# neeek2303/EMOPortraits

Hardware: AMD Instinct MI355X
Metric: reenactment frames/sec @512x512, 1-src->N-driver (higher is better)
Workload: dtype f32

## Files before the change

emoportraits_amd/csrc/conv_inst_f16x2_up2.hip:

```cpp
#include "conv_dispatch.h"
#include "conv_igemm_bf16x3.h"
#include "conv_split_pair_common.h"

struct ConvCfgUp2 {
  static constexpr int BM = 64, TM = 2, TP = 2, KC = 16, NPL = 2;
  static constexpr int TRL = 2, TWL = 64;
  static constexpr int PR = TRL + 2, NQ = TWL / 4, NQ1 = NQ + 1;
  static constexpr int SUB = ((PR * NQ1 + 4 + 11) / 16) * 16 + 4;
  static constexpr int CHS = 4 * SUB, NG = 2, QPG = 128, NHQ = 2 * PR;
  static constexpr int WPLANE = 2 * BM;
  static constexpr int WTAP = NPL * WPLANE;
  static constexpr int WST = 8 * WTAP;
  static constexpr int WST_BYTES = WST * 16;
  static constexpr int PPL = NG * CHS, PBUF = NPL * PPL;
  static constexpr int OFF_P = 0, OFF_W = 2 * PBUF, OFF_SCT = OFF_W + 2 * WST;
  static constexpr int SCT = 1024;
  static constexpr int OFF_BIAS_F = OFF_SCT * 4 + 2 * SCT;
  static constexpr int EPI_CS = 4 * 132 + 4;
  static constexpr int LDS_BYTES = (OFF_BIAS_F + BM) * 4;
  static_assert(32 * EPI_CS <= OFF_SCT * 4, "the epilogue image lives in the patch and kernel buffers");
  static_assert(WST_BYTES == 32 * 1024, "eight 1 KiB pieces per wave and half-stage");
  static_assert(PR * NQ + NHQ <= QPG, "one interior quad or one halo pixel per thread and stage");
  static_assert(LDS_BYTES <= 160 * 1024, "LDS");
};

__global__ __launch_bounds__(256) __attribute__((amdgpu_waves_per_eu(1, 1)))
void conv_igemm_f16x2_up2_kernel(const ConvArgs a) {
  using Cfg = ConvCfgUp2;
  using opx8 = halfx8;
  constexpr int NPL = 2, NPROD = 3;
  constexpr int BM = Cfg::BM, TM = Cfg::TM, TP = Cfg::TP, KC = Cfg::KC;
  constexpr int PR = Cfg::PR, NQ = Cfg::NQ, NQ1 = Cfg::NQ1, SUB = Cfg::SUB, CHS = Cfg::CHS, QPG = Cfg::QPG;
  constexpr int NHQ = Cfg::NHQ, PPL = Cfg::PPL, PBUF = Cfg::PBUF;
  constexpr bool UPS = false;
  constexpr int TW = Cfg::TWL, TWS = Cfg::TWL;

  extern __shared__ __attribute__((aligned(16))) float smem[];

  const int tid = threadIdx.x;
  const int lane = tid & 63;
  const int wave = __builtin_amdgcn_readfirstlane(tid >> 6);
  const int half = lane >> 5, l32 = lane & 31;
  const int wq = wave & 1;
  const int p0 = (wave >> 1) * TP * 32;
  float sat_m = 0.0f;

  const int HW = a.H * a.W;
  const bool has_affine = a.scale != nullptr;
  const float in_scale = a.in_scale;
  constexpr float CLAMP_HI = 65504.0f;
  const float clamp_lo = a.relu_in ? 0.0f : -CLAMP_HI;
  const int nst = a.n_cchunks;
  const int nptiles = a.tiles_x * a.tiles_y;

  const int q_u = tid % QPG;
  const int q_g = __builtin_amdgcn_readfirstlane(tid / QPG);
  const bool is_quad = q_u < PR * NQ;
  const int hq = q_u - PR * NQ;
  const bool is_halo = !is_quad && hq < NHQ;
  const int h_side = hq & 1;
  const int q_r = is_quad ? q_u / NQ : (is_halo ? hq >> 1 : 0);
  const int q_c = is_quad ? q_u - q_r * NQ : 0;
  int q_slb[4];
#pragma unroll
  for (int i = 0; i < 4; ++i) {
    const int dump = q_g * CHS + i * SUB + PR * NQ1 + (q_u & 3);
    const int own = is_quad ? q_g * CHS + i * SUB + q_r * NQ1 + q_c : q_g * CHS + h_side * SUB + q_r * NQ1 + NQ;
    q_slb[i] = ((is_quad || (is_halo && i == (h_side ? 0 : 3))) ? own : dump) * 16;
  }

  floatx16 acc_lo[2][TM][TP], acc_hi[2][TM][TP];

  const int q8 = a.n_work >> 3, r8 = a.n_work & 7;
  const int xcd = blockIdx.x & 7;
  const int n_mine = q8 + (xcd < r8 ? 1 : 0);
  const int l_base = xcd < r8 ? xcd * (q8 + 1) : r8 * (q8 + 1) + (xcd - r8) * q8;
  const int l_stride = (gridDim.x + 7) >> 3;
#define EMO_U_WPTR(c_, k_, p_) (reinterpret_cast<const char*>(a.wpk) + ((long)((c_) * nst + (k_)) * 2 + (p_)) * Cfg::WST_BYTES)

  const int a_off = (half * BM + l32) * 16;
  EMO_P_DECLARE_B_OFF()

  const char* const lds_c = reinterpret_cast<const char*>(smem);
  char* const lds_w = reinterpret_cast<char*>(smem);
  opx8 fa_[2][NPL][TM], fb_[2][NPL][TP];
#define EMO_U_LOAD_FRAGS_PLANE(set_, pl_, hb_, pbyte_, a_, b_)                                        \
  {                                                                                                   \
    _Pragma("unroll") for (int i = 0; i < TM; ++i)                                                    \
      fa_[set_][pl_][i] = *reinterpret_cast<const opx8*>(lds_c + a_off + (Cfg::OFF_W + (hb_) * Cfg::WST + \
          ((wq * 4 + (a_) * 2 + (b_)) * NPL + (pl_)) * Cfg::WPLANE + i * 32) * 16);                   \
    _Pragma("unroll") for (int j = 0; j < TP; ++j)                                                    \
      fb_[set_][pl_][j] = *reinterpret_cast<const opx8*>(lds_c + (EMO_P_B_OFF(j, (hb_) + (a_), wq + (b_)) + (pbyte_)) + ((pl_) * PPL) * 16); \
  }

  float* const sct = smem + Cfg::OFF_SCT * 4;
  const unsigned smem_lds = (unsigned)(size_t)(__attribute__((address_space(3))) char*)reinterpret_cast<char*>(smem);
  const unsigned lane16 = (unsigned)lane * 16u;

  floatx4 qv[8];
  float q_lo, q_hi;
  int q_tix;
  floatx4 q_sc, q_sh;
  opx8 cv_h, cv_m;
  emo_intx4 xrs = emo_raw_buffer(a.x);
  unsigned usoff[8];
#pragma unroll
  for (int u = 0; u < 8; ++u) usoff[u] = (unsigned)__builtin_amdgcn_readfirstlane((int)((unsigned)u * (unsigned)HW * 4u));
  unsigned lq_off = 0;
  bool lq_ok = false;
  unsigned q_vo;
#define EMO_U_ISSUE_BEGIN(st_)                                                                        \
  {                                                                                                   \
    const int c0_ = (st_) * KC + q_g * 8;                                                             \
    const bool cv_ = c0_ < a.Cin;                                                                     \
    const int cs_ = cv_ ? c0_ : 0;                                                                    \
    const bool keep_ = lq_ok && cv_;                                                                  \
    q_lo = keep_ ? clamp_lo : 0.0f;                                                                   \
    q_hi = keep_ ? CLAMP_HI : 0.0f;                                                                   \
    q_vo = lq_off + (unsigned)cs_ * (unsigned)HW * 4u;                                                \
    q_tix = (has_affine ? cs_ : (cs_ & (Cfg::SCT - 1))) >> 2;                                         \
  }
#define EMO_U_ISSUE_LOADS(u0_, u1_)                                                                   \
  { _Pragma("unroll") for (int u = (u0_); u < (u1_); u += 2) emo_bload4x2_pinned(xrs, q_vo, usoff[u], usoff[u + 1], qv[u], qv[u + 1]); }
#define EMO_U_HALF_TABLE(hf_)                                                                         \
  {                                                                                                   \
    const floatx4* t4_ = reinterpret_cast<const floatx4*>(sct) + q_tix + (hf_);                       \
    q_sc = t4_[0]; q_sh = t4_[Cfg::SCT / 4];                                                          \
  }
#define EMO_U_TOUCH_QUAD() { _Pragma("unroll") for (int u = 0; u < 8; ++u) emo_touch4(qv[u]); }
#define EMO_U_CONV_PIXEL(pbyte_, i_)                                                                  \
  {                                                                                                   \
    _Pragma("unroll") for (int hf_ = 0; hf_ < 2; ++hf_) {                                             \
      EMO_U_HALF_TABLE(hf_)                                                                           \
      float t_[4];                                                                                    \
      _Pragma("unroll") for (int k = 0; k < 4; ++k)                                                   \
        t_[k] = __fmaf_rn(qv[4 * hf_ + k][i_], q_sc[k], q_sh[k]);                                     \
      sat_m = __builtin_fmaxf(__builtin_fmaxf(sat_m, __builtin_fabsf(t_[0])), __builtin_fabsf(t_[1])); \
      sat_m = __builtin_fmaxf(__builtin_fmaxf(sat_m, __builtin_fabsf(t_[2])), __builtin_fabsf(t_[3])); \
      _Pragma("unroll") for (int k = 0; k < 4; k += 2)                                                \
        emo_split_f16x2_pair(__builtin_amdgcn_fmed3f(t_[k], q_lo, q_hi), __builtin_amdgcn_fmed3f(t_[k + 1], q_lo, q_hi), \
                             cv_h, cv_m, 4 * hf_ + k);                                                \
    }                                                                                                 \
    char* d_ = lds_w + (q_slb[i_] + (pbyte_));                                                        \
    *reinterpret_cast<opx8*>(d_) = cv_h;                                                              \
    *reinterpret_cast<opx8*>(d_ + PPL * 16) = cv_m;                                                   \
  }
#define EMO_U_DMA_PIECE(ptr_, wb_, k_)                                                                \
  {                                                                                                   \
    const int j_ = wave + 4 * (k_);                                                                   \
    emo_dma16_pinned_s((ptr_) + j_ * 1024, lane16, smem_lds + (unsigned)((Cfg::OFF_W + (wb_) * Cfg::WST) * 16 + j_ * 1024)); \
  }

  constexpr int PA3[3] = {1, 0, 0}, PB3[3] = {0, 1, 0};
  constexpr int NTE = Cfg::SCT / 256;

  for (int idx8 = blockIdx.x >> 3; idx8 < n_mine; idx8 += l_stride) {
    const int l_ = l_base + idx8;
    const int cotile = __builtin_amdgcn_readfirstlane(l_ % a.n_cotiles);
    const int rest_ = l_ / a.n_cotiles;
    const int it_n = __builtin_amdgcn_readfirstlane(rest_ / nptiles);
    const int lt_ = rest_ - it_n * nptiles;
    const int x0 = __builtin_amdgcn_readfirstlane((lt_ % a.tiles_x) * Cfg::TWL);
    const int y0 = __builtin_amdgcn_readfirstlane((lt_ / a.tiles_x) * Cfg::TRL);
    {
      const int q_y_ = y0 - 1 + q_r;
      const int q_x_ = is_quad ? x0 + 4 * q_c : (h_side ? x0 + TWS : x0 - 4);
      lq_ok = (is_quad || is_halo) && (unsigned)q_y_ < (unsigned)a.H && q_x_ >= 0 && q_x_ < a.W;
      lq_off = lq_ok ? (unsigned)(q_y_ * a.W + q_x_) * 4u : 0u;
    }
    xrs = emo_raw_buffer(a.x + (long)it_n * a.Cin * HW);

#pragma unroll
    for (int u = 0; u < 8; ++u) asm volatile("" : "=v"(qv[u]));
    asm volatile("" : "=v"(cv_h));
    asm volatile("" : "=v"(cv_m));
    {
      const char* const w0_ = EMO_U_WPTR(cotile, 0, 0);
#pragma unroll
      for (int k = 0; k < 8; ++k) EMO_U_DMA_PIECE(w0_, 0, k)
      const char* const w1_ = EMO_U_WPTR(cotile, 0, 1);
      EMO_U_DMA_PIECE(w1_, 1, 0)
      EMO_U_DMA_PIECE(w1_, 1, 1)
    }
    EMO_U_ISSUE_BEGIN(0)
    EMO_U_ISSUE_LOADS(0, 8)
#pragma unroll
    for (int k = 0; k < NTE; ++k) {
      const int c = tid + 256 * k;
      if (c < min(a.Cin, Cfg::SCT)) {
        const bool real = has_affine;
        sct[c] = (real ? a.scale[(long)it_n * a.Cin + c] : 1.0f) * in_scale;
        sct[Cfg::SCT + c] = (real ? a.shift[(long)it_n * a.Cin + c] : 0.0f) * in_scale;
      }
    }
    if (tid < BM) smem[Cfg::OFF_BIAS_F + tid] = a.bias != nullptr ? a.bias[cotile * BM + tid] : 0.0f;
    EMO_P_WAIT(0);
    EMO_U_TOUCH_QUAD()
    __syncthreads();
#pragma unroll
    for (int i = 0; i < 4; ++i) EMO_U_CONV_PIXEL(Cfg::OFF_P * 16, i)
    EMO_U_ISSUE_BEGIN(nst > 1 ? 1 : 0)
    EMO_U_ISSUE_LOADS(0, 8)
    EMO_P_BARRIER(0);
    EMO_U_TOUCH_QUAD()

#pragma unroll
    for (int c = 0; c < 2; ++c)
#pragma unroll
      for (int i = 0; i < TM; ++i)
#pragma unroll
        for (int j = 0; j < TP; ++j)
#pragma unroll
          for (int r = 0; r < 16; ++r) { acc_lo[c][i][j][r] = 0.0f; acc_hi[c][i][j][r] = 0.0f; }
#pragma unroll
    for (int pl = 0; pl < NPL; ++pl) EMO_U_LOAD_FRAGS_PLANE(0, pl, 0, Cfg::OFF_P * 16, 0, 0)
    int pp = 0;
    for (int cg = 0; cg < nst; ++cg) {
      const int pcur_b = (Cfg::OFF_P + pp * PBUF) * 16, pnxt_b = (Cfg::OFF_P + (pp ^ 1) * PBUF) * 16;
      const bool last_ = cg + 1 >= nst;
#pragma unroll
      for (int h = 0; h < 2; ++h) {
        const bool have1_ = h == 0 || !last_, have2_ = !last_;
        const char* const dma1 = EMO_U_WPTR(cotile, h == 0 ? cg : cg + 1, h ^ 1);
        const char* const dma2 = EMO_U_WPTR(cotile, cg + 1, h);
        if (EMO_CONV_SETPRIO) __builtin_amdgcn_s_setprio(1);
#pragma unroll
        for (int gs = 0; gs < 4; ++gs) {
          const int fcur = (h * 4 + gs) & 1, fnxt = fcur ^ 1;
          if (gs == 3) { EMO_P_BARRIER(0); }
          if (gs == 3 && h == 1) EMO_U_TOUCH_QUAD()
          if (gs == 0 && h == 1) {
            const int tgt_ = cg + 2 < nst ? cg + 2 : nst - 1;
            EMO_U_ISSUE_BEGIN(tgt_)
          }
          __builtin_amdgcn_sched_barrier(0);
          {
            const int an = gs < 3 ? (gs + 1) >> 1 : 0, bn = gs < 3 ? (gs + 1) & 1 : 0;
            const int hbn = gs < 3 ? h : h ^ 1;
            const int pbn = (gs == 3 && h == 1) ? pnxt_b : pcur_b;
#pragma unroll
            for (int pl = 0; pl < NPL; ++pl) {
              EMO_U_LOAD_FRAGS_PLANE(fnxt, pl, hbn, pbn, an, bn)
              if (gs < 3 && have1_) EMO_U_DMA_PIECE(dma1, h ^ 1, 2 + 2 * gs + pl)
              if (gs == 3 && have2_) EMO_U_DMA_PIECE(dma2, h, pl)
              if (h == 1 && gs == 0) EMO_U_ISSUE_LOADS(2 * pl, 2 * pl + 2)
              if (h == 1 && gs > 0 && gs < 3 && pl == 0) EMO_U_ISSUE_LOADS(2 + 2 * gs, 4 + 2 * gs)
            }
          }
          if (h == 0) EMO_U_CONV_PIXEL(pnxt_b, gs)
#pragma unroll
          for (int p = 0; p < NPROD; ++p) {
            const int pa = PA3[p], pb = PB3[p];
#pragma unroll
            for (int i = 0; i < TM; ++i)
#pragma unroll
              for (int j = 0; j < TP; ++j) {
                floatx16& acc_ = (pa == 0 && pb == 0) ? acc_lo[h][i][j] : acc_hi[h][i][j];
                acc_ = __builtin_amdgcn_mfma_f32_32x32x16_f16(fb_[fcur][pb][j], fa_[fcur][pa][i], acc_, 0, 0, 0);
              }
          }
          __builtin_amdgcn_sched_barrier(0);
        }
        if (EMO_CONV_SETPRIO) __builtin_amdgcn_s_setprio(0);
      }
      pp ^= 1;
    }

    EMO_P_WAIT(0);
    __syncthreads();
    const bool want_stats = a.gn_stats != nullptr;
    const int Ho = a.Hl, Wo = a.Wl;
    const unsigned oplane = (unsigned)Ho * Wo;
    const int tiles_xo = Wo / 64;
    const int ec = tid >> 4, eu = tid & 15;
#pragma unroll
    for (int i = 0; i < TM; ++i) {
#pragma unroll
      for (int p = 0; p < 2; ++p)
#pragma unroll
        for (int j = 0; j < TP; ++j)
#pragma unroll
          for (int r = 0; r < 16; ++r) {
            const float v = (emo_acc_read(acc_lo[p][i][j][r]) + emo_acc_read(acc_hi[p][i][j][r])) * a.out_scale;
            const int m = (r >> 2) * 8 + half * 4 + (r & 3);
            const int hr = 2 * (wave >> 1) + p, col = 2 * (j * 32 + m) + wq;
            smem[l32 * Cfg::EPI_CS + hr * 132 + col] = v;
          }
      __syncthreads();
#pragma unroll
      for (int cc = 0; cc < 2; ++cc) {
        const int c = cc * 16 + ec;
        const int co = cotile * BM + i * 32 + c;
        const float bs = smem[Cfg::OFF_BIAS_F + i * 32 + c];
        float* const obase = a.out + ((long)it_n * a.Cout + co) * oplane;
        float s_[2] = {0.0f, 0.0f};
        floatx4 v_[4][2];
#pragma unroll
        for (int hr = 0; hr < 4; ++hr)
#pragma unroll
          for (int k = 0; k < 2; ++k) {
            floatx4 v = *reinterpret_cast<const floatx4*>(smem + c * Cfg::EPI_CS + hr * 132 + 4 * eu + 64 * k);
            v = v + floatx4{bs, bs, bs, bs};
            v_[hr][k] = v;
            float* const op = obase + (unsigned)(2 * y0 + hr) * Wo + (2 * x0 + 4 * eu + 64 * k);
            if (EMO_CONV_NT_STORE) __builtin_nontemporal_store(v, reinterpret_cast<floatx4*>(op));
            else *reinterpret_cast<floatx4*>(op) = v;
            s_[k] += (v[0] + v[1]) + (v[2] + v[3]);
          }
        if (want_stats) {
          emo_row16_sum_n<2>(s_);
          float m2_[2] = {0.0f, 0.0f};
#pragma unroll
          for (int k = 0; k < 2; ++k) {
            s_[k] *= 1.0f / 256.0f;
#pragma unroll
            for (int hr = 0; hr < 4; ++hr)
#pragma unroll
              for (int e = 0; e < 4; ++e) {
                const float d = v_[hr][k][e] - s_[k];
                m2_[k] = __fmaf_rn(d, d, m2_[k]);
              }
          }
          emo_row16_sum_n<2>(m2_);
          if (eu == 0) {
#pragma unroll
            for (int k = 0; k < 2; ++k) {
              const int ptile = (y0 >> 1) * tiles_xo + (x0 >> 5) + k;
              reinterpret_cast<float2*>(a.gn_stats)[((long)it_n * (oplane / 256) + ptile) * a.Cout + co] = make_float2(s_[k], m2_[k]);
            }
          }
        }
      }
      __syncthreads();
    }
  }
  if (a.sat_flag != nullptr && sat_m > 65504.0f) *a.sat_flag = 1;
#undef EMO_U_WPTR
#undef EMO_U_LOAD_FRAGS_PLANE
#undef EMO_U_ISSUE_BEGIN
#undef EMO_U_ISSUE_LOADS
#undef EMO_U_HALF_TABLE
#undef EMO_U_TOUCH_QUAD
#undef EMO_U_CONV_PIXEL
#undef EMO_U_DMA_PIECE
}

int conv_f16x2_up2_launch(ConvArgs a, hipStream_t s) {
  using Cfg = ConvCfgUp2;
  if (a.KD != 1 || a.D != 1 || a.ksplit != 1 || a.res != nullptr || a.act != EMO_ACT_NONE || a.run_if != nullptr) return EMO_ERR_UNSUPPORTED;
  if (a.Cout % Cfg::BM || a.Cin % 8 || (a.scale && a.Cin > Cfg::SCT)) return EMO_ERR_UNSUPPORTED;
  if (a.W % Cfg::TWL || a.H % Cfg::TRL) return EMO_ERR_UNSUPPORTED;
  if ((reinterpret_cast<unsigned long long>(a.x) & 15ull) || (reinterpret_cast<unsigned long long>(a.out) & 15ull)) return EMO_ERR_ALIGN;
  if ((unsigned long long)a.Cin * a.H * a.W * 4ull >= (1ull << 32) || (long)a.Hl * a.Wl >= (1l << 31)) return EMO_ERR_UNSUPPORTED;
  const long nt = (long)(a.W / Cfg::TWL) * (a.H / Cfg::TRL);
  const int cot = a.Cout / Cfg::BM;
  if (a.N > 65535 || nt * cot * a.N > 0x7fffffffL) return EMO_ERR_UNSUPPORTED;
  auto kern = conv_igemm_f16x2_up2_kernel;
  const int rc = emo_raise_dynamic_lds(kern);
  if (rc != EMO_OK) return rc;
  a.tiles_x = a.W / Cfg::TWL;
  a.tiles_y = a.H / Cfg::TRL;
  a.tiles_z = 1;
  a.n_cchunks = (a.Cin + Cfg::KC - 1) / Cfg::KC;
  a.stages_per_split = a.n_cchunks;
  a.partial = nullptr;
  a.cot0 = 0;
  a.n_cotiles = cot;
  a.n_work = (int)(nt * cot * a.N);
  const int ncu = emo_cu_count();
  const int grid = a.n_work > ncu ? ncu : a.n_work;
  hipLaunchKernelGGL(kern, dim3((unsigned)grid), dim3(256), (size_t)Cfg::LDS_BYTES, s, a);
  return emo_launch_status();
}
```

Measured before the change: 399.0.

## Chain consecutive work items in up2 conv to prefetch next tile's weights and patches

The persistent up2 conv kernel now decodes the next work item and, when it shares the same batch image, prefetches that item's first-stage weights, input patch loads and bias during the last stage and epilogue of the current item, skipping the cold prologue. The epilogue image moves to a separate LDS region so it no longer overwrites the buffers the successor needs. Next-stage input loads are also issued earlier, inside the first half-stage. This adds LDS footprint, extra address logic and optional timing instrumentation, and chaining applies only when consecutive items share an image.

```diff
diff --git a/emoportraits_amd/csrc/conv_inst_f16x2_up2.hip b/emoportraits_amd/csrc/conv_inst_f16x2_up2.hip
--- a/emoportraits_amd/csrc/conv_inst_f16x2_up2.hip
+++ b/emoportraits_amd/csrc/conv_inst_f16x2_up2.hip
@@ -1,6 +1,13 @@
 #include "conv_dispatch.h"
 #include "conv_igemm_bf16x3.h"
 #include "conv_split_pair_common.h"
+
+#ifndef EMO_UP2_CHAIN
+#define EMO_UP2_CHAIN 1
+#endif
+#ifndef EMO_UP2_LOADS_EARLY
+#define EMO_UP2_LOADS_EARLY 1
+#endif
 
 struct ConvCfgUp2 {
   static constexpr int BM = 64, TM = 2, TP = 2, KC = 16, NPL = 2;
@@ -13,12 +20,15 @@
   static constexpr int WST = 8 * WTAP;
   static constexpr int WST_BYTES = WST * 16;
   static constexpr int PPL = NG * CHS, PBUF = NPL * PPL;
-  static constexpr int OFF_P = 0, OFF_W = 2 * PBUF, OFF_SCT = OFF_W + 2 * WST;
   static constexpr int SCT = 1024;
+  static constexpr int OFF_P = 0, OFF_W = 2 * PBUF, OFF_SCT = OFF_W + WST;
+  static constexpr int WSTRIDE = WST + (2 * SCT + BM) / 4;
   static constexpr int OFF_BIAS_F = OFF_SCT * 4 + 2 * SCT;
   static constexpr int EPI_CS = 4 * 132 + 4;
-  static constexpr int LDS_BYTES = (OFF_BIAS_F + BM) * 4;
-  static_assert(32 * EPI_CS <= OFF_SCT * 4, "the epilogue image lives in the patch and kernel buffers");
+  static constexpr int OFF_IMG_F = (OFF_W + WSTRIDE) * 4;
+  static constexpr int LDS_BYTES = (OFF_IMG_F + 32 * EPI_CS) * 4;
+  static_assert(OFF_IMG_F >= OFF_BIAS_F + BM, "the epilogue image spares the patch buffers, W[0], the tables and the bias: a chained successor's");
+  static_assert(32 * EPI_CS * 4 >= WST_BYTES, "W[1] lies inside the image's allocation");
   static_assert(WST_BYTES == 32 * 1024, "eight 1 KiB pieces per wave and half-stage");
   static_assert(PR * NQ + NHQ <= QPG, "one interior quad or one halo pixel per thread and stage");
   static_assert(LDS_BYTES <= 160 * 1024, "LDS");
@@ -87,7 +97,7 @@
 #define EMO_U_LOAD_FRAGS_PLANE(set_, pl_, hb_, pbyte_, a_, b_)                                        \
   {                                                                                                   \
     _Pragma("unroll") for (int i = 0; i < TM; ++i)                                                    \
-      fa_[set_][pl_][i] = *reinterpret_cast<const opx8*>(lds_c + a_off + (Cfg::OFF_W + (hb_) * Cfg::WST + \
+      fa_[set_][pl_][i] = *reinterpret_cast<const opx8*>(lds_c + a_off + (Cfg::OFF_W + (hb_) * Cfg::WSTRIDE + \
           ((wq * 4 + (a_) * 2 + (b_)) * NPL + (pl_)) * Cfg::WPLANE + i * 32) * 16);                   \
     _Pragma("unroll") for (int j = 0; j < TP; ++j)                                                    \
       fb_[set_][pl_][j] = *reinterpret_cast<const opx8*>(lds_c + (EMO_P_B_OFF(j, (hb_) + (a_), wq + (b_)) + (pbyte_)) + ((pl_) * PPL) * 16); \
@@ -148,62 +158,126 @@
 #define EMO_U_DMA_PIECE(ptr_, wb_, k_)                                                                \
   {                                                                                                   \
     const int j_ = wave + 4 * (k_);                                                                   \
-    emo_dma16_pinned_s((ptr_) + j_ * 1024, lane16, smem_lds + (unsigned)((Cfg::OFF_W + (wb_) * Cfg::WST) * 16 + j_ * 1024)); \
+    emo_dma16_pinned_s((ptr_) + j_ * 1024, lane16, smem_lds + (unsigned)((Cfg::OFF_W + (wb_) * Cfg::WSTRIDE) * 16 + j_ * 1024)); \
   }
 
   constexpr int PA3[3] = {1, 0, 0}, PB3[3] = {0, 1, 0};
   constexpr int NTE = Cfg::SCT / 256;
 
+#define EMO_U_DECODE(P_, L_)                                                                          \
+  {                                                                                                   \
+    const int l_ = (L_);                                                                              \
+    P_##cotile = __builtin_amdgcn_readfirstlane(l_ % a.n_cotiles);                                    \
+    const int rest_ = l_ / a.n_cotiles;                                                               \
+    P_##n = __builtin_amdgcn_readfirstlane(rest_ / nptiles);                                          \
+    const int lt_ = rest_ - P_##n * nptiles;                                                          \
+    P_##x0 = __builtin_amdgcn_readfirstlane((lt_ % a.tiles_x) * Cfg::TWL);        \
+    P_##y0 = __builtin_amdgcn_readfirstlane((lt_ / a.tiles_x) * Cfg::TRL);                            \
+  }
+#define EMO_U_CURSOR_OF(P_, ok_, off_)                                                                \
+  {                                                                                                   \
+    const int q_y_ = P_##y0 - 1 + q_r;                                                                \
+    const int q_x_ = is_quad ? P_##x0 + 4 * q_c : (h_side ? P_##x0 + TWS : P_##x0 - 4);               \
+    ok_ = (is_quad || is_halo) && (unsigned)q_y_ < (unsigned)a.H && q_x_ >= 0 && q_x_ < a.W;          \
+    off_ = ok_ ? (unsigned)(q_y_ * a.W + q_x_) * 4u : 0u;                                             \
+  }
+#define EMO_U_NEXT_STAGE_BEGIN()                                                                      \
+  {                                                                                                   \
+    const bool sw_ = chain_out && cg + 2 == nst;                                                      \
+    const int tgt_ = (chain_out && cg + 2 >= nst) ? cg + 2 - nst : (cg + 2 < nst ? cg + 2 : nst - 1); \
+    lq_ok = sw_ ? nxq_ok : lq_ok;                                                                     \
+    lq_off = sw_ ? nxq_off : lq_off;                                                                  \
+    EMO_U_ISSUE_BEGIN(tgt_)                                                                           \
+  }
+#if EMO_S_TIMING == 2
+#define EMO_U_LOOP_BARRIER(n_)                                                                        \
+  {                                                                                                   \
+    const unsigned long long b0_ = __builtin_amdgcn_s_memtime();                                      \
+    asm volatile("s_waitcnt vmcnt(%0) lgkmcnt(0)" ::"n"(n_) : "memory");                              \
+    const unsigned long long b1_ = __builtin_amdgcn_s_memtime();                                      \
+    asm volatile("s_waitcnt lgkmcnt(0)\n\ts_barrier" ::: "memory");                                  \
+    const unsigned long long b2_ = __builtin_amdgcn_s_memtime();                                      \
+    asm volatile("s_waitcnt lgkmcnt(0)" ::: "memory");                                                \
+    tw_wait += b1_ - b0_; tw_bar += b2_ - b1_; ++tw_n;                                                \
+  }
+#else
+#define EMO_U_LOOP_BARRIER(n_) EMO_P_BARRIER(n_)
+#endif
+
+  constexpr bool CHAIN = EMO_UP2_CHAIN != 0, LOADS_EARLY = EMO_UP2_LOADS_EARLY != 0;
+  float te_b = 0.0f;
+  bool chained_in = false;
+  int pp = 0;
   for (int idx8 = blockIdx.x >> 3; idx8 < n_mine; idx8 += l_stride) {
-    const int l_ = l_base + idx8;
-    const int cotile = __builtin_amdgcn_readfirstlane(l_ % a.n_cotiles);
-    const int rest_ = l_ / a.n_cotiles;
-    const int it_n = __builtin_amdgcn_readfirstlane(rest_ / nptiles);
-    const int lt_ = rest_ - it_n * nptiles;
-    const int x0 = __builtin_amdgcn_readfirstlane((lt_ % a.tiles_x) * Cfg::TWL);
-    const int y0 = __builtin_amdgcn_readfirstlane((lt_ / a.tiles_x) * Cfg::TRL);
+#if EMO_S_TIMING
+    unsigned long long tstamp[12];
+    for (int k = 0; k < 12; ++k) tstamp[k] = 0;
+    unsigned long long tw_wait = 0, tw_bar = 0, tw_n = 0;
+#endif
+    EMO_S_STAMP(0)
+    int cotile, it_n, x0, y0;
     {
-      const int q_y_ = y0 - 1 + q_r;
-      const int q_x_ = is_quad ? x0 + 4 * q_c : (h_side ? x0 + TWS : x0 - 4);
-      lq_ok = (is_quad || is_halo) && (unsigned)q_y_ < (unsigned)a.H && q_x_ >= 0 && q_x_ < a.W;
-      lq_off = lq_ok ? (unsigned)(q_y_ * a.W + q_x_) * 4u : 0u;
+      int it_cotile, it_x0, it_y0;
+      EMO_U_DECODE(it_, l_base + idx8)
+      cotile = it_cotile; x0 = it_x0; y0 = it_y0;
+    }
+    int nx_cotile = 0, nx_n = 0, nx_x0 = 0, nx_y0 = 0;
+    bool chain_out = false, nxq_ok = false;
+    unsigned nxq_off = 0;
+    if (CHAIN && idx8 + l_stride < n_mine) {
+      EMO_U_DECODE(nx_, l_base + idx8 + l_stride)
+      chain_out = nx_n == it_n && nst >= 2;
+      EMO_U_CURSOR_OF(nx_, nxq_ok, nxq_off)
     }
     xrs = emo_raw_buffer(a.x + (long)it_n * a.Cin * HW);
-
-#pragma unroll
-    for (int u = 0; u < 8; ++u) asm volatile("" : "=v"(qv[u]));
     asm volatile("" : "=v"(cv_h));
     asm volatile("" : "=v"(cv_m));
-    {
-      const char* const w0_ = EMO_U_WPTR(cotile, 0, 0);
-#pragma unroll
-      for (int k = 0; k < 8; ++k) EMO_U_DMA_PIECE(w0_, 0, k)
+    if (CHAIN && chained_in) {
+      if (tid < BM) smem[Cfg::OFF_BIAS_F + tid] = te_b;
       const char* const w1_ = EMO_U_WPTR(cotile, 0, 1);
       EMO_U_DMA_PIECE(w1_, 1, 0)
       EMO_U_DMA_PIECE(w1_, 1, 1)
-    }
-    EMO_U_ISSUE_BEGIN(0)
-    EMO_U_ISSUE_LOADS(0, 8)
-#pragma unroll
-    for (int k = 0; k < NTE; ++k) {
-      const int c = tid + 256 * k;
-      if (c < min(a.Cin, Cfg::SCT)) {
-        const bool real = has_affine;
-        sct[c] = (real ? a.scale[(long)it_n * a.Cin + c] : 1.0f) * in_scale;
-        sct[Cfg::SCT + c] = (real ? a.shift[(long)it_n * a.Cin + c] : 0.0f) * in_scale;
-      }
-    }
-    if (tid < BM) smem[Cfg::OFF_BIAS_F + tid] = a.bias != nullptr ? a.bias[cotile * BM + tid] : 0.0f;
-    EMO_P_WAIT(0);
-    EMO_U_TOUCH_QUAD()
-    __syncthreads();
-#pragma unroll
-    for (int i = 0; i < 4; ++i) EMO_U_CONV_PIXEL(Cfg::OFF_P * 16, i)
-    EMO_U_ISSUE_BEGIN(nst > 1 ? 1 : 0)
-    EMO_U_ISSUE_LOADS(0, 8)
-    EMO_P_BARRIER(0);
-    EMO_U_TOUCH_QUAD()
-
+      EMO_P_BARRIER(40);
+    } else {
+      {
+        int it_x0 = x0, it_y0 = y0;
+        EMO_U_CURSOR_OF(it_, lq_ok, lq_off)
+      }
+#pragma unroll
+      for (int u = 0; u < 8; ++u) asm volatile("" : "=v"(qv[u]));
+      {
+        const char* const w0_ = EMO_U_WPTR(cotile, 0, 0);
+#pragma unroll
+        for (int k = 0; k < 8; ++k) EMO_U_DMA_PIECE(w0_, 0, k)
+        const char* const w1_ = EMO_U_WPTR(cotile, 0, 1);
+        EMO_U_DMA_PIECE(w1_, 1, 0)
+        EMO_U_DMA_PIECE(w1_, 1, 1)
+      }
+      EMO_U_ISSUE_BEGIN(0)
+      EMO_U_ISSUE_LOADS(0, 8)
+#pragma unroll
+      for (int k = 0; k < NTE; ++k) {
+        const int c = tid + 256 * k;
+        if (c < min(a.Cin, Cfg::SCT)) {
+          const bool real = has_affine;
+          sct[c] = (real ? a.scale[(long)it_n * a.Cin + c] : 1.0f) * in_scale;
+          sct[Cfg::SCT + c] = (real ? a.shift[(long)it_n * a.Cin + c] : 0.0f) * in_scale;
+        }
+      }
+      if (tid < BM) smem[Cfg::OFF_BIAS_F + tid] = a.bias != nullptr ? a.bias[cotile * BM + tid] : 0.0f;
+      EMO_P_WAIT(0);
+      EMO_U_TOUCH_QUAD()
+      __syncthreads();
+#pragma unroll
+      for (int i = 0; i < 4; ++i) EMO_U_CONV_PIXEL(Cfg::OFF_P * 16, i)
+      EMO_U_ISSUE_BEGIN(nst > 1 ? 1 : 0)
+      EMO_U_ISSUE_LOADS(0, 8)
+      EMO_P_BARRIER(0);
+      EMO_U_TOUCH_QUAD()
+      pp = 0;
+    }
+
+    EMO_S_STAMP(1)
 #pragma unroll
     for (int c = 0; c < 2; ++c)
 #pragma unroll
@@ -212,27 +286,28 @@
         for (int j = 0; j < TP; ++j)
 #pragma unroll
           for (int r = 0; r < 16; ++r) { acc_lo[c][i][j][r] = 0.0f; acc_hi[c][i][j][r] = 0.0f; }
-#pragma unroll
-    for (int pl = 0; pl < NPL; ++pl) EMO_U_LOAD_FRAGS_PLANE(0, pl, 0, Cfg::OFF_P * 16, 0, 0)
-    int pp = 0;
+    {
+      const int pb0_ = (Cfg::OFF_P + pp * PBUF) * 16;
+#pragma unroll
+      for (int pl = 0; pl < NPL; ++pl) EMO_U_LOAD_FRAGS_PLANE(0, pl, 0, pb0_, 0, 0)
+    }
     for (int cg = 0; cg < nst; ++cg) {
       const int pcur_b = (Cfg::OFF_P + pp * PBUF) * 16, pnxt_b = (Cfg::OFF_P + (pp ^ 1) * PBUF) * 16;
       const bool last_ = cg + 1 >= nst;
 #pragma unroll
       for (int h = 0; h < 2; ++h) {
-        const bool have1_ = h == 0 || !last_, have2_ = !last_;
-        const char* const dma1 = EMO_U_WPTR(cotile, h == 0 ? cg : cg + 1, h ^ 1);
-        const char* const dma2 = EMO_U_WPTR(cotile, cg + 1, h);
+        const bool past_ = last_ && chain_out;
+        const bool have1_ = CHAIN || h == 0 || !last_, have2_ = !last_ || (CHAIN && h == 0);
+        const int ce_ = past_ ? nx_cotile : cotile, ke_ = last_ ? (chain_out ? 0 : nst - 1) : cg + 1;
+        const char* const dma1 = h == 0 ? EMO_U_WPTR(cotile, cg, 1) : EMO_U_WPTR(ce_, ke_, 0);
+        const char* const dma2 = EMO_U_WPTR(ce_, ke_, h);
         if (EMO_CONV_SETPRIO) __builtin_amdgcn_s_setprio(1);
 #pragma unroll
         for (int gs = 0; gs < 4; ++gs) {
           const int fcur = (h * 4 + gs) & 1, fnxt = fcur ^ 1;
-          if (gs == 3) { EMO_P_BARRIER(0); }
+          if (gs == 3) { EMO_U_LOOP_BARRIER(0); }
           if (gs == 3 && h == 1) EMO_U_TOUCH_QUAD()
-          if (gs == 0 && h == 1) {
-            const int tgt_ = cg + 2 < nst ? cg + 2 : nst - 1;
-            EMO_U_ISSUE_BEGIN(tgt_)
-          }
+          if (!LOADS_EARLY && gs == 0 && h == 1) EMO_U_NEXT_STAGE_BEGIN()
           __builtin_amdgcn_sched_barrier(0);
           {
             const int an = gs < 3 ? (gs + 1) >> 1 : 0, bn = gs < 3 ? (gs + 1) & 1 : 0;
@@ -243,11 +318,15 @@
               EMO_U_LOAD_FRAGS_PLANE(fnxt, pl, hbn, pbn, an, bn)
               if (gs < 3 && have1_) EMO_U_DMA_PIECE(dma1, h ^ 1, 2 + 2 * gs + pl)
               if (gs == 3 && have2_) EMO_U_DMA_PIECE(dma2, h, pl)
-              if (h == 1 && gs == 0) EMO_U_ISSUE_LOADS(2 * pl, 2 * pl + 2)
-              if (h == 1 && gs > 0 && gs < 3 && pl == 0) EMO_U_ISSUE_LOADS(2 + 2 * gs, 4 + 2 * gs)
+              if (!LOADS_EARLY && h == 1 && gs == 0) EMO_U_ISSUE_LOADS(2 * pl, 2 * pl + 2)
+              if (!LOADS_EARLY && h == 1 && gs > 0 && gs < 3 && pl == 0) EMO_U_ISSUE_LOADS(2 + 2 * gs, 4 + 2 * gs)
             }
           }
           if (h == 0) EMO_U_CONV_PIXEL(pnxt_b, gs)
+          if (LOADS_EARLY && h == 0 && gs == 3) {
+            EMO_U_NEXT_STAGE_BEGIN()
+            EMO_U_ISSUE_LOADS(0, 8)
+          }
 #pragma unroll
           for (int p = 0; p < NPROD; ++p) {
             const int pa = PA3[p], pb = PB3[p];
@@ -266,8 +345,14 @@
       pp ^= 1;
     }
 
+    EMO_S_STAMP(2)
     EMO_P_WAIT(0);
+    EMO_S_STAMP(5)
     __syncthreads();
+    EMO_S_STAMP(6)
+    EMO_S_STAMP(7)
+    float* const img = smem + Cfg::OFF_IMG_F;
+    if (CHAIN && chain_out && tid < BM) te_b = a.bias != nullptr ? a.bias[nx_cotile * BM + tid] : 0.0f;
     const bool want_stats = a.gn_stats != nullptr;
     const int Ho = a.Hl, Wo = a.Wl;
     const unsigned oplane = (unsigned)Ho * Wo;
@@ -284,7 +369,7 @@
             const float v = (emo_acc_read(acc_lo[p][i][j][r]) + emo_acc_read(acc_hi[p][i][j][r])) * a.out_scale;
             const int m = (r >> 2) * 8 + half * 4 + (r & 3);
             const int hr = 2 * (wave >> 1) + p, col = 2 * (j * 32 + m) + wq;
-            smem[l32 * Cfg::EPI_CS + hr * 132 + col] = v;
+            img[l32 * Cfg::EPI_CS + hr * 132 + col] = v;
           }
       __syncthreads();
 #pragma unroll
@@ -299,7 +384,7 @@
         for (int hr = 0; hr < 4; ++hr)
 #pragma unroll
           for (int k = 0; k < 2; ++k) {
-            floatx4 v = *reinterpret_cast<const floatx4*>(smem + c * Cfg::EPI_CS + hr * 132 + 4 * eu + 64 * k);
+            floatx4 v = *reinterpret_cast<const floatx4*>(img + c * Cfg::EPI_CS + hr * 132 + 4 * eu + 64 * k);
             v = v + floatx4{bs, bs, bs, bs};
             v_[hr][k] = v;
             float* const op = obase + (unsigned)(2 * y0 + hr) * Wo + (2 * x0 + 4 * eu + 64 * k);
@@ -331,11 +416,42 @@
           }
         }
       }
-      __syncthreads();
-    }
+      if (i == 0) {
+        EMO_S_STAMP(8)
+        __syncthreads();
+      }
+    }
+    EMO_S_STAMP(9)
+#if EMO_S_TIMING
+    EMO_S_STAMP(3)
+    asm volatile("s_waitcnt vmcnt(0)" ::: "memory");
+    EMO_S_STAMP(4)
+    {
+      const int ep_L_ = l_base + idx8;
+      if (tid == 0 && ep_L_ < EMO_S_TLOG_N) {
+        unsigned long long* t_ = emo_s_tlog + (long)ep_L_ * EMO_S_TLOG_W;
+#pragma unroll
+        for (int k = 0; k < 12; ++k) t_[k] = tstamp[k];
+        t_[12] = (unsigned long long)__builtin_amdgcn_s_getreg((31 << 11) | 4);
+        t_[13] = (unsigned long long)__builtin_amdgcn_s_getreg((31 << 11) | 20);
+        t_[14] = (unsigned long long)blockIdx.x;
+        t_[15] = (unsigned long long)(chained_in ? 1 : 0);
+      }
+      if (EMO_S_TIMING == 2 && lane == 0 && ep_L_ < EMO_S_TLOG_N / 8) {
+        unsigned long long* w_ = emo_s_tlog + ((long)EMO_S_TLOG_N / 4 + (long)ep_L_ * 4 + wave) * EMO_S_TLOG_W;
+        w_[0] = tw_wait; w_[1] = tw_bar; w_[2] = tw_n; w_[3] = tstamp[2] - tstamp[1];
+      }
+    }
+#endif
+    __syncthreads();
+    chained_in = chain_out;
   }
   if (a.sat_flag != nullptr && sat_m > 65504.0f) *a.sat_flag = 1;
 #undef EMO_U_WPTR
+#undef EMO_U_DECODE
+#undef EMO_U_CURSOR_OF
+#undef EMO_U_NEXT_STAGE_BEGIN
+#undef EMO_U_LOOP_BARRIER
 #undef EMO_U_LOAD_FRAGS_PLANE
 #undef EMO_U_ISSUE_BEGIN
 #undef EMO_U_ISSUE_LOADS
@@ -372,3 +488,11 @@
   hipLaunchKernelGGL(kern, dim3((unsigned)grid), dim3(256), (size_t)Cfg::LDS_BYTES, s, a);
   return emo_launch_status();
 }
+
+#if EMO_S_TIMING
+extern "C" int emo_debug_conv_timing_up2(unsigned long long* host_out, int n_items) {
+  if (!host_out || n_items < 0 || n_items > EMO_S_TLOG_N) return EMO_ERR_BAD_ARG;
+  if (hipDeviceSynchronize() != hipSuccess) return EMO_ERR_BAD_ARG;
+  return hipMemcpyFromSymbol(host_out, HIP_SYMBOL(emo_s_tlog), (size_t)n_items * EMO_S_TLOG_W * sizeof(unsigned long long)) == hipSuccess ? EMO_OK : EMO_ERR_BAD_ARG;
+}
+#endif
```

Result: faster. 404.4, median of 6 (+1.4%).
